# iamwangyabin/hardnetNas

Hardware: AMD Instinct MI355X
Metric: Mpatches/s (32×32→128-D) at 1/2/4/8 MI355X; HPatches FPR95 parity (higher is better)
Workload: dtype bf16x3; 1 GPU; Stock HardNet forward, 262144 synthetic 32x32 patches per GPU; model=hardnet, global_batch=262144, per_gpu_batch=262144, parallelism=dp1

## Files before the change

### hardnetnas_amd/csrc/hn_api.hip

```cpp
#include "hardnet_mi355x.h"
#include "hn_internal.h"

#include <algorithm>
#include <cmath>
#include <cstdlib>
#include <cstring>
#include <map>
#include <mutex>
#include <string>
#include <utility>
#include <vector>

static thread_local std::string g_err;

static int env_int(const char* name, int dflt) {
  const char* e = std::getenv(name);
  return e ? std::atoi(e) : dflt;
}

void hn_read_knobs(HnKnobs* k) {
  *k = HnKnobs{};
  k->c12_cfg = env_int("HN_C12_CFG", 15);
  k->head = std::getenv("HN_HEAD_V1") ? 1 : env_int("HN_HEAD", 4);
  k->head_pf = env_int("HN_HEAD_PF", 1) != 0;
  k->fdl_valu = std::getenv("HN_FDL_VALU") != nullptr;
  k->naive_pw = std::getenv("HN_NAIVE_PW") != nullptr;
  k->naive_dw = std::getenv("HN_NAIVE_DW") != nullptr;
  k->no_skipfuse = std::getenv("HN_NO_SKIPFUSE") != nullptr;
  k->no_irfskip = std::getenv("HN_NO_IRFSKIP") != nullptr;
  k->pairdist_valu = std::getenv("HN_PAIRDIST_VALU") != nullptr;
  k->pairdist_reg = env_int("HN_PAIRDIST_REG", 0) != 0;
  k->pairdist_spread = env_int("HN_PAIRDIST_SPREAD", 1) != 0;
  k->front_fold = env_int("HN_FRONT_FOLD", 0) != 0;
  k->u8_apart = env_int("HN_U8_APART", 0) != 0;
  k->front_xch3 = env_int("HN_FRONT_XCH3", 0) != 0;
  k->no_mpfront = env_int("HN_NO_MPFRONT", 0) != 0;
  k->pipeline = env_int("HN_PIPELINE", 0) != 0;

  k->train_splitk = std::max(32, env_int("HN_TRAIN_SPLITK", 1024)) / 32 * 32;
  k->train_f32 = env_int("HN_TRAIN_F32", 17) & 255;
#ifdef HN_EXPERIMENTS
  k->c12_abl = env_int("HN_C12_ABL", 0) & 4095;
  k->c12w_pd = env_int("HN_C12W_PD", 11);
  k->dbg = env_int("HN_DEBUG", 0);
  k->head_abl = env_int("HN_HEAD_ABL", 0);
  k->w4_abl = env_int("HN_W4_ABL", 0);
  k->pairdist_abl = env_int("HN_PAIRDIST_ABL", 0);
  k->irf3 = env_int("HN_IRF3", 0) != 0;
#endif
}

static thread_local const HnKnobs* tl_knobs = nullptr;

const HnKnobs& hn_knobs() {
  if (tl_knobs) return *tl_knobs;
  static std::once_flag once;
  static HnKnobs process;
  std::call_once(once, [] { hn_read_knobs(&process); });
  return process;
}

namespace {
struct KnobScope {
  const HnKnobs* prev;
  explicit KnobScope(const HnKnobs* k) : prev(tl_knobs) { tl_knobs = k; }
  ~KnobScope() { tl_knobs = prev; }
};
}

hipError_t hn_resident_blocks(const void* fn, int nthreads, int lds, int* resident) {
  static std::mutex mu;
  static std::map<std::pair<const void*, int>, int> cache;
  int dev = 0;
  hipError_t e = hipGetDevice(&dev);
  if (e != hipSuccess) return e;
  std::lock_guard<std::mutex> lock(mu);
  auto it = cache.find({fn, dev});
  if (it != cache.end()) {
    *resident = it->second;
    return hipSuccess;
  }
  if (lds > 0 && (e = hipFuncSetAttribute(fn, hipFuncAttributeMaxDynamicSharedMemorySize, lds)) != hipSuccess)
    return e;
  int per_cu = 0, cus = 0;
  if ((e = hipOccupancyMaxActiveBlocksPerMultiprocessor(&per_cu, fn, nthreads, lds)) != hipSuccess) return e;
  if ((e = hipDeviceGetAttribute(&cus, hipDeviceAttributeMultiprocessorCount, dev)) != hipSuccess) return e;
  const int r = std::max(1, per_cu) * std::max(1, cus);
  cache[{fn, dev}] = r;
  *resident = r;
  return hipSuccess;
}

static int fail(int code, const std::string& msg) {
  g_err = msg;
  return code;
}

#define HIPCHK(x)                                                                          \
  do {                                                                                     \
    hipError_t e_ = (x);                                                                   \
    if (e_ != hipSuccess)                                                                  \
      return fail(HN_ERR_HIP, std::string(#x) + ": " + hipGetErrorString(e_));             \
  } while (0)

const HnOpSpec kHnOps[17] = {
    {"skip", 1, 0, 0, 0, 0},        {"ir_k3_e1", 0, 1, 3, 1, 0},    {"ir_k3_e3", 0, 3, 3, 1, 0},
    {"ir_k3_s4", 0, 4, 3, 4, 0},    {"ir_k5_e1", 0, 1, 5, 1, 0},    {"ir_k5_e3", 0, 3, 5, 1, 0},
    {"ir_k5_s4", 0, 4, 5, 4, 0},    {"ir_k3_e1_se", 0, 1, 3, 1, 1}, {"ir_k3_e3_se", 0, 3, 3, 1, 1},
    {"ir_k3_s4_se", 0, 4, 3, 4, 1}, {"ir_k5_e1_se", 0, 1, 5, 1, 1}, {"ir_k5_e3_se", 0, 3, 5, 1, 1},
    {"ir_k5_s4_se", 0, 4, 5, 4, 1}, {"ir_k3_s2", 0, 1, 3, 2, 0},    {"ir_k5_s2", 0, 1, 5, 2, 0},
    {"ir_k3_s2_se", 0, 1, 3, 2, 1}, {"ir_k5_s2_se", 0, 1, 5, 2, 1},
};

namespace {

using OpSpec = HnOpSpec;
const OpSpec* const kOps = kHnOps;

struct NasLayer {
  int op = 0, cin = 0, cout = 0, stride = 1, hin = 0, hout = 0;
  int skip = 0, e = 1, k = 3, g = 1, se = 0, mid = 0, semid = 0;
  int skip_conv = 0;
  float *pw_w = nullptr, *pw_b = nullptr, *dw_w = nullptr, *dw_b = nullptr;
  float *pwl_w = nullptr, *pwl_b = nullptr;
  float *se_w1 = nullptr, *se_b1 = nullptr, *se_w2 = nullptr, *se_b2 = nullptr;
  uint16_t* front_a = nullptr;
  uint16_t* front_pwl16 = nullptr;
  float* front_b = nullptr;
  uint16_t *irf_pw_a = nullptr, *irf_pwl_a = nullptr;
  uint16_t* skip_a = nullptr;
  float* irf_pw_b = nullptr;
};

struct Cursor {
  const float* p;
  size_t n, i = 0;
  bool ok = true;
  const float* take(size_t k) {
    if (i + k > n) {
      ok = false;
      return nullptr;
    }
    const float* r = p + i;
    i += k;
    return r;
  }
};

uint16_t f2bf(float x) {
  uint32_t u;
  std::memcpy(&u, &x, 4);
  u += 0x7FFFu + ((u >> 16) & 1u);
  return (uint16_t)(u >> 16);
}
float bf2f(uint16_t b) {
  uint32_t u = (uint32_t)b << 16;
  float f;
  std::memcpy(&f, &u, 4);
  return f;
}

struct Folded {
  std::vector<float> w, b;
};
Folded fold(const float* w, size_t per_out, int cout, const float* gamma, const float* beta,
            const float* mean, const float* var, float eps) {
  Folded f;
  f.w.resize((size_t)cout * per_out);
  f.b.resize(cout);
  for (int n = 0; n < cout; ++n) {
    const double sc = (gamma ? (double)gamma[n] : 1.0) / std::sqrt((double)var[n] + (double)eps);
    for (size_t j = 0; j < per_out; ++j)
      f.w[(size_t)n * per_out + j] = (float)((double)w[(size_t)n * per_out + j] * sc);
    f.b[n] = (float)((beta ? (double)beta[n] : 0.0) - (double)mean[n] * sc);
  }
  return f;
}
// ... 1734 lines not shown
```

### hardnetnas_amd/csrc/hn_internal.h

```cpp
#pragma once
#include <hip/hip_runtime.h>

#include <algorithm>
#include <type_traits>

#include "hardnet_mi355x.h"

struct HnKnobs {
  int c12_cfg = 15;
  int head = 4;
  bool head_pf = true;
  bool fdl_valu = false;
  bool naive_pw = false;
  bool naive_dw = false;
  bool no_skipfuse = false;
  bool no_irfskip = false;
  bool pairdist_valu = false;
  bool pairdist_reg = false;
  bool pairdist_spread = true;
  bool front_fold = false;
  bool u8_apart = false;
  bool front_xch3 = false;
  bool no_mpfront = false;
  bool pipeline = false;
  bool irf3 = false;
  int train_splitk = 1024;
  int train_f32 = 17;
  int c12w_pd = 11;
  int c12_abl = 0;
  int head_abl = 0;
  int w4_abl = 0;
  int pairdist_abl = 0;
  int dbg = 0;
};
void hn_read_knobs(HnKnobs* k);
const HnKnobs& hn_knobs();

hipError_t hn_resident_blocks(const void* fn, int nthreads, int lds, int* resident);

struct HardnetDev {
  float* stem_w = nullptr;
  float* stem_b = nullptr;
  void* wpack[7] = {};
  float* bias[7] = {};
  void* c12_w1 = nullptr;
  void* c12_w2 = nullptr;
  void* c12_w1w = nullptr;
  void* wino[7] = {};
  void* wino1[7] = {};
  void* wino4[7] = {};
};
struct HnU8In {
  const uint8_t* in;
  int resize;
  int normalize;
  float mean, stdv;
};
hipError_t hn_launch_c12(const float* in, float* out, const HardnetDev& d, int P, float eps,
                         hipStream_t st, const HnU8In* u8 = nullptr);

hipError_t hn_launch_stem(const float* in, float* out, const float* w, const float* b, int P,
                          bool norm, float eps, hipStream_t st);
using HnConvLaunch = hipError_t (*)(const HardnetDev& d, const float* in, float* out, int P, float eps,
                                    hipStream_t st);
struct HnConvRow {
  int layer, variant;
  HnConvLaunch launch;
};
template <int N>
constexpr const HnConvRow* hn_find_row(const HnConvRow (&rows)[N], int layer, int variant) {
  for (const HnConvRow& r : rows)
    if (r.layer == layer && r.variant == variant) return &r;
  return nullptr;
}
template <int N>
constexpr bool hn_rows_unique(const HnConvRow (&rows)[N]) {
  for (int i = 0; i < N; ++i)
    if (hn_find_row(rows, rows[i].layer, rows[i].variant) != &rows[i]) return false;
  return true;
}
const HnConvRow* hn_hardnet_conv_row(int layer, int variant);
const HnConvRow* hn_wino1_conv_row(int layer, int variant);
const HnConvRow* hn_wino_conv_row(int layer, int variant);
bool hn_hardnet_variant_ok(int layer, int variant);

template <auto Kernel, int NTHR, int SMEM, class... Args>
hipError_t hn_launch_persistent(int tiles, hipStream_t st, Args... args) {
  int resident = 0;
  const hipError_t e = hn_resident_blocks(reinterpret_cast<const void*>(Kernel), NTHR, SMEM, &resident);
  if (e != hipSuccess) return e;
  const int grid = std::min(tiles, resident);
  if (grid <= 0) return hipSuccess;
  hipLaunchKernelGGL(Kernel, dim3(grid), dim3(NTHR), SMEM, st, args...);
  return hipGetLastError();
}

using HnC12Launch = hipError_t (*)(const float* in, float* out, const HardnetDev& d, int P, float eps,
                                   hipStream_t st, const HnU8In* u8);
constexpr int kAnyPd = -1;
struct HnC12Row {
  int cfg, abl, pd;
  HnC12Launch launch;
};
constexpr int kC12Wino = 14;
constexpr int kC12Split = 15;
template <int N>
constexpr const HnC12Row* hn_find_row(const HnC12Row (&rows)[N], int cfg, int abl, int pd) {
  for (const HnC12Row& r : rows)
    if (r.cfg == cfg && r.abl == abl && (r.pd == pd || r.pd == kAnyPd)) return &r;
  return nullptr;
}
template <int N>
constexpr bool hn_rows_unique(const HnC12Row (&rows)[N]) {
  for (int i = 0; i < N; ++i)
    if (hn_find_row(rows, rows[i].cfg, rows[i].abl, rows[i].pd) != &rows[i]) return false;
  return true;
}
const HnC12Row* hn_c12_row(int cfg, int abl, int pd);
const HnC12Row* hn_c12w_row(int cfg, int abl, int pd);
bool hn_c12_cfg_ok(int cfg, int abl, int pd);
template <auto Kernel, auto Base, int NTHR>
hipError_t hn_c12_launch(const void* w1, const float* in, float* out, const HardnetDev& d, int P, float eps,
                         hipStream_t st, const HnU8In* u8) {
  int resident = 0;
  const hipError_t e = hn_resident_blocks(reinterpret_cast<const void*>(Base), NTHR, 0, &resident);
  if (e != hipSuccess) return e;
  const int grid = (int)std::min<long>((long)P, resident);
  const void* src = u8 ? u8->in : static_cast<const void*>(in);
  hipLaunchKernelGGL(Kernel, dim3(grid), dim3(NTHR), 0, st, src, out, d.stem_w, d.stem_b, static_cast<const uint4*>(w1),
                     d.bias[1], static_cast<const uint4*>(d.c12_w2), d.bias[2], P, eps, u8 ? u8->mean : 0.f,
                     u8 ? u8->stdv : 1.f, u8 ? u8->normalize : 0);
  return hipGetLastError();
}
template <class F>
hipError_t hn_with_u8(const HnU8In* u8, F&& f) {
  if (!u8) return f(std::integral_constant<int, -1>{});
  switch (u8->resize) {
    case HN_RESIZE_NONE: return f(std::integral_constant<int, HN_RESIZE_NONE>{});
    case HN_RESIZE_CV2_LINEAR: return f(std::integral_constant<int, HN_RESIZE_CV2_LINEAR>{});
    case HN_RESIZE_PIL_BILINEAR: return f(std::integral_constant<int, HN_RESIZE_PIL_BILINEAR>{});
  }
  return hipErrorInvalidValue;
}
constexpr int kHeadSplitMaxP = 16384;
constexpr int head_split(int K) { return K / 128; }
hipError_t hn_launch_head(const float* a, float* out, const void* wp, const float* bias, int P,
                          int K, float l2eps, hipStream_t st, bool f16 = false, float* part = nullptr);
int hn_conv_lds_bytes(int layer);
hipError_t hn_launch_conv_raw(int layer, const void* wp, const float* zero_bias, const float* in, float* out,
                              int P, hipStream_t st);
int hn_wino1_lds_bytes(int layer);

hipError_t hn_launch_pw(const float* in, float* out, const float* wt, const float* bias,
                        const float* res, long npix, int cin, int cout, int groups, bool relu,
                        int shuffle_g, hipStream_t st);
hipError_t hn_launch_dw(const float* in, float* out, const float* wd, const float* bias, int P,
                        int hin, int c, int k, int s, hipStream_t st);
hipError_t hn_launch_maxpool(const float* in, float* out, int P, int hin, int c, hipStream_t st);
bool hn_skip_s2_supported(int hin, int cin, int cout);
hipError_t hn_launch_skip_s2(const float* in, float* out, const float* wt, const float* bias, int P, int hin,
                             int cin, int cout, hipStream_t st);
hipError_t hn_launch_se(float* y, const float* w1, const float* b1, const float* w2,
                        const float* b2, int P, int hw, int c, int mid, hipStream_t st);
hipError_t hn_launch_nas_head(const float* a, float* out, const float* wt, const float* bias,
// ... 156 lines not shown
```

### hardnetnas_amd/csrc/hn_wino1.hip

```cpp
#include "hn_common.h"
#include "hn_internal.h"

namespace {

template <int CIN, int COUT, int H, int NP, int WM, int WN, bool CST>
struct W1Cfg {
  static constexpr int TR = H;
  static constexpr int NTX = H / 2;
  static constexpr int BM = NP * TR * NTX;
  static constexpr int MT = BM / WM / 32, NT = COUT / WN / 32;
  static constexpr int NTOT = COUT / 32, NCC = CIN / 32;
  static constexpr int XROW = NTX * 64;
  static constexpr int RS = 4 * XROW;
  static constexpr int PS = TR * RS;
  static constexpr int ZROW = NP * PS;
  static constexpr int PLANE = ZROW + RS;
  static constexpr int BUF = 2 * PLANE;
  static constexpr int NWC = WM * WN, NWP = 4, NTHR = (NWC + NWP) * 64, PTHR = NWP * 64;
  static constexpr int UNITS = NP * TR * NTX * 4;
  static_assert(64 % (4 * NTX) == 0 && PTHR % (4 * NTX) == 0, "a row's units share one wave");
  static constexpr int UPT = (UNITS + PTHR - 1) / PTHR;
  static constexpr bool DEEP = UPT <= 2;
  static constexpr int SROW = 36;
  static constexpr int SCR_OFF = 2 * BUF;
  static constexpr int SCR = CST ? 32 * SROW * 4 : 0;
  static constexpr int BIAS_OFF = SCR_OFF + NWC * SCR;
  static constexpr int SMEM = BIAS_OFF + COUT * 4;
  static constexpr int NKS = 24;
  static constexpr unsigned CHUNK_BYTES = NKS * NTOT * 2 * 64 * 16;
  static_assert(SMEM <= 160 * 1024, "LDS");
  static_assert(MT >= 1 && NT >= 1 && MT * WM * 32 == BM && NT * WN * 32 == COUT, "tiling");
  static_assert((TR * NTX) % 32 == 0 && 32 % NTX == 0, "an M tile = 32 / NTX whole rows of one patch");
  static_assert(RS % 256 == 0, "image rows on 256-byte boundaries (the bank-conflict argument)");
};

template <int... I, class F>
HN_DEV void static_for_seq(std::integer_sequence<int, I...>, F&& f) {
  (f(std::integral_constant<int, I>{}), ...);
}
template <int N, class F>
HN_DEV void static_for(F&& f) {
  static_for_seq(std::make_integer_sequence<int, N>{}, f);
}

constexpr int w1_lo3(int g) { return g == 0 ? 0 : g == 1 ? 6 : g == 2 ? 11 : 16; }
constexpr int w1_fold_valu(bool first, int kx, int g) {
  if (kx == 11 && g >= 3) return 2 * (w1_lo3(g - 2) - w1_lo3(g - 3));
  if (kx == 12 && g < 3) return 2 * (w1_lo3(g + 1) - w1_lo3(g));
  if (kx == 18 || kx == 19 || (kx == 0 && !first)) return g < 5 ? 3 : 1;
  if (kx == 23 && g >= 3) return w1_lo3(g - 2) - w1_lo3(g - 3);
  return 0;
}

template <int CIN, int COUT, int H, int NP, int WM, int WN, bool CST, int WD = 3, int ABL = 0>
__global__ __launch_bounds__((WM * WN + 4) * 64) void k_conv_w1(const float* __restrict__ in, float* __restrict__ out,
                                                                const uint4* __restrict__ wp,
                                                                const float* __restrict__ bias, int P) {
  using C = W1Cfg<CIN, COUT, H, NP, WM, WN, CST>;
  constexpr int TR = C::TR;
  extern __shared__ __attribute__((aligned(16))) char smem[];
  const int tid = threadIdx.x, lane = tid & 63;
  const int wave = __builtin_amdgcn_readfirstlane(tid >> 6);
  const bool producer = wave >= C::NWC;
  const int r = lane & 31, h = lane >> 5;
  const int nwg = gridDim.x, rb = xcd_remap(blockIdx.x, nwg);
  const int ntiles = (P + NP - 1) / NP;
  const int my_tiles = rb < ntiles ? (ntiles - 1 - rb) / nwg + 1 : 0;
  const int NS = my_tiles * C::NCC;
  if (NS == 0) return;
  char* const buf0 = smem;
  char* const buf1 = smem + C::BUF;
  auto tile_of = [&](int s) { return (rb + (s / C::NCC) * nwg) * NP; };

  const int ptid = tid - C::NWC * 64;
  float4 pf[C::UPT][6], pf2[C::UPT][6];
  constexpr unsigned PATCH_BYTES = (unsigned)H * H * CIN * 4, OOB = 0x80000000u;
  auto produce_loads = [&](int s, float4 (&d)[C::UPT][6]) {
    const bool live = s < NS;
    const int p0 = live ? tile_of(s) : 0;
    const int cc = s % C::NCC;
    const int nval = !live ? 0 : P - p0 < NP ? P - p0 : NP;
    const __amdgpu_buffer_rsrc_t rs = make_rsrc(in + (size_t)p0 * H * H * CIN, (unsigned)nval * PATCH_BYTES);
#pragma unroll
    for (int k = 0; k < C::UPT; ++k) {
      const int u = ptid + k * C::PTHR;
      const int g = u & 3, t = (u >> 2) % C::NTX, rest = (u >> 2) / C::NTX;
      const int y = rest % TR, np = rest / TR;
      const bool rowok = C::UNITS % C::PTHR == 0 || u < C::UNITS;
#pragma unroll
      for (int j = 0; j < 3; ++j) {
        const int x = 2 * t - 1 + j;
        const bool ok = rowok && (j < 2 || t == C::NTX - 1) && (unsigned)x < (unsigned)H;
        const unsigned vo = ok ? (unsigned)(((np * H + y) * H + x) * CIN + cc * 32 + g * 8) * 4u : OOB;
        d[k][2 * j] = __builtin_bit_cast(float4, buf_load16(rs, vo, 0));
        d[k][2 * j + 1] = __builtin_bit_cast(float4, buf_load16(rs, vo, 16));
      }
    }
  };
  auto shfl4 = [&](const float4& v) {
    return make_float4(__shfl_down(v.x, 4, 64), __shfl_down(v.y, 4, 64), __shfl_down(v.z, 4, 64),
                       __shfl_down(v.w, 4, 64));
  };
  auto produce_write = [&](char* dst, const float4 (&d)[C::UPT][6]) {
#pragma unroll
    for (int k = 0; k < C::UPT; ++k) {
      const int u = ptid + k * C::PTHR;
      const int g = u & 3, t = (u >> 2) % C::NTX, rest = (u >> 2) / C::NTX;
      const int y = rest % TR, np = rest / TR;
      const bool last = t == C::NTX - 1;
      const float4 z = make_float4(0.f, 0.f, 0.f, 0.f);
      float4 dd[4][2];
#pragma unroll
      for (int i = 0; i < 2; ++i) {
        const float4 n0 = shfl4(d[k][i]), n1 = shfl4(d[k][2 + i]);
        dd[0][i] = d[k][i];
        dd[1][i] = d[k][2 + i];
        dd[2][i] = last ? d[k][4 + i] : n0;
        dd[3][i] = last ? z : n1;
      }
      if (C::UNITS % C::PTHR == 0 || u < C::UNITS) {
        const int off = np * C::PS + y * C::RS + t * 64 + 16 * (g ^ ((y + 1) & 3));
#pragma unroll
        for (int xi = 0; xi < 4; ++xi) {
          float4 v[2];
#pragma unroll
          for (int i = 0; i < 2; ++i) {
            const float4 d0 = dd[0][i], d1 = dd[1][i], d2 = dd[2][i], d3 = dd[3][i];
            if (xi == 0) v[i] = make_float4(d0.x - d2.x, d0.y - d2.y, d0.z - d2.z, d0.w - d2.w);
            if (xi == 1) v[i] = make_float4(d1.x + d2.x, d1.y + d2.y, d1.z + d2.z, d1.w + d2.w);
            if (xi == 2) v[i] = make_float4(d2.x - d1.x, d2.y - d1.y, d2.z - d1.z, d2.w - d1.w);
            if (xi == 3) v[i] = make_float4(d1.x - d3.x, d1.y - d3.y, d1.z - d3.z, d1.w - d3.w);
          }
          uint4 hi, lo;
          split8(v[0], v[1], hi, lo);
          *reinterpret_cast<uint4*>(dst + off + xi * C::XROW) = hi;
          *reinterpret_cast<uint4*>(dst + C::PLANE + off + xi * C::XROW) = lo;
        }
      }
    }
  };

  for (int i = tid; i < 4 * C::RS / 16; i += C::NTHR) {
    const int q = i / (C::RS / 16), o = (i % (C::RS / 16)) * 16;
    *reinterpret_cast<uint4*>(smem + (q >> 1) * C::BUF + (q & 1) * C::PLANE + C::ZROW + o) = make_uint4(0, 0, 0, 0);
  }
  if constexpr ((ABL & 64) != 0) {
    if (!producer) __builtin_amdgcn_s_setprio(1);
  }
  if constexpr ((ABL & 128) != 0) {
    if (producer) __builtin_amdgcn_s_setprio(1);
  }
  if (producer) {
    if constexpr ((ABL & 1) != 0) {
#pragma unroll 1
      for (int s = 0; s <= NS; ++s) __syncthreads();
      return;
    }
    produce_loads(0, pf);
    produce_write(buf0, pf);
    produce_loads(1, pf);
    __syncthreads();
    if constexpr (!C::DEEP) {
#pragma unroll 1
      for (int s = 0; s < NS; ++s) {
        produce_write((s & 1) ? buf0 : buf1, pf);
        produce_loads(s + 2, pf);
        __syncthreads();
      }
    } else {
#pragma unroll 1
      for (int s = 0; s < NS; s += 2) {
        produce_loads(s + 2, pf2);
        produce_write(buf1, pf);
        __syncthreads();
        if (s + 1 >= NS) break;
        produce_loads(s + 3, pf);
        produce_write(buf0, pf2);
        __syncthreads();
      }
    }
    return;
  }

  for (int i = tid; i < COUT; i += C::NWC * 64) reinterpret_cast<float*>(smem + C::BIAS_OFF)[i] = bias[i];
  __syncthreads();
  if constexpr ((ABL & 16) != 0) {
#pragma unroll 1
    for (int s = 0; s < NS; ++s) __syncthreads();
    return;
  }
  const int wm = wave / WN, wn = wave % WN;
  const float* const sbias = reinterpret_cast<const float*>(smem + C::BIAS_OFF);
  int ylr[C::MT], vo[C::MT][3][2];
#pragma unroll
  for (int mt = 0; mt < C::MT; ++mt) {
    const int m = (wm * C::MT + mt) * 32 + r;
    const int np = m / (TR * C::NTX), rem = m % (TR * C::NTX);
    ylr[mt] = rem / C::NTX;
#pragma unroll
    for (int ky = 0; ky < 3; ++ky) {
      const int wr = ylr[mt] + ky;
      const int rowb = (wr >= 1 && wr <= TR) ? np * C::PS + (wr - 1) * C::RS : C::ZROW;
#pragma unroll
      for (int ks = 0; ks < 2; ++ks) {
        vo[mt][ky][ks] = rowb + (rem % C::NTX) * 64 + 16 * ((2 * ks + h) ^ (wr & 3));
        asm volatile("" : "+v"(vo[mt][ky][ks]));
      }
    }
  }
  const __amdgpu_buffer_rsrc_t wr_ = make_rsrc(wp, C::NCC * C::CHUNK_BYTES);
  const unsigned wvoff = (wn * C::NT * 2 * 64 + lane) * 16;
  static_assert(C::MT * C::NT == 2, "the fold schedule below is written for two accumulator tiles per wave");
  f32x16 y0a[2], y1a[2], ma[2];

  auto load_b = [&](int cc, int kx, uint4 (&dst)[C::NT][2]) {
#pragma unroll
    for (int nt = 0; nt < C::NT; ++nt) {
      const unsigned k = cc * C::CHUNK_BYTES + (((ABL & 4) ? 0 : kx) * C::NTOT + nt) * 2 * 64 * 16;
      dst[nt][0] = buf_load16(wr_, wvoff, k);
      dst[nt][1] = buf_load16(wr_, wvoff, k + 64 * 16);
    }
  };
  static_assert(C::NKS % WD == 0, "the weight ring runs on across stages");
  uint4 bq[WD][C::NT][2];
#pragma unroll
  for (int k = 0; k + 1 < WD; ++k) load_b(0, k, bq[k]);

  auto sadd = [](float a, float b) {
    float v = a + b;
    asm("" : "+v"(v));
    return v;
  };
  auto ssub = [](float a, float b) {
    float v = a - b;
    asm("" : "+v"(v));
    return v;
  };
  auto fold = [&](auto first_, auto kx_, auto g_) {
    constexpr bool first = decltype(first_)::value;
    constexpr int kx = decltype(kx_)::value, g = decltype(g_)::value;
    if constexpr ((kx == 11 && g >= 3) || (kx == 12 && g < 3)) {
      constexpr int j = kx == 11 ? 0 : 1, g3 = kx == 11 ? g - 3 : g;
#pragma unroll
      for (int i = w1_lo3(g3); i < w1_lo3(g3 + 1); ++i) {
        y0a[j][i] = sadd(y0a[j][i], ma[j][i]);
        y1a[j][i] = sadd(first ? 0.f : y1a[j][i], ma[j][i]);
      }
    } else if constexpr (kx == 18 || kx == 19) {
#pragma unroll
      for (int i = 3 * g; i < 3 * g + 3 && i < 16; ++i) y0a[kx - 18][i] = sadd(y0a[kx - 18][i], ma[kx - 18][i]);
    } else if constexpr (kx == 23 && g >= 3) {
#pragma unroll
      for (int i = w1_lo3(g - 3); i < w1_lo3(g - 2); ++i) y1a[0][i] = ssub(y1a[0][i], ma[0][i]);
    } else if constexpr (kx == 0 && !first) {
#pragma unroll
      for (int i = 3 * g; i < 3 * g + 3 && i < 16; ++i) y1a[1][i] = ssub(y1a[1][i], ma[1][i]);
    }
  };

  auto stage = [&](auto first_, int s, int cc, int ccn) {
    constexpr bool FIRST = decltype(first_)::value;
    const char* cur = (s & 1) ? buf1 : buf0;
    uint4 aq[2][C::MT][2];
    auto load_a = [&](int kx, uint4 (&dst)[C::MT][2]) {
      const int xi = kx / 6, ky = (kx % 6) >> 1, ks = kx & 1;
#pragma unroll
      for (int mt = 0; mt < C::MT; ++mt) {
        const char* pa = cur + vo[mt][ky][ks];
        dst[mt][0] = *reinterpret_cast<const uint4*>(pa + xi * C::XROW);
        dst[mt][1] = *reinterpret_cast<const uint4*>(pa + (C::PLANE + xi * C::XROW));
      }
    };
    load_a(0, aq[0]);
    static_for<C::NKS>([&](auto kx_) {
      constexpr int kx = decltype(kx_)::value, xi = kx / 6;
      if constexpr ((ABL & 32) != 0) {
      } else if constexpr (kx + WD - 1 < C::NKS)
        load_b(cc, kx + WD - 1, bq[(kx + WD - 1) % WD]);
      else
        load_b(ccn, kx + WD - 1 - C::NKS, bq[(kx + WD - 1) % WD]);
      if constexpr (kx + 1 < C::NKS) load_a(kx + 1, aq[(kx + 1) & 1]);
      __builtin_amdgcn_sched_barrier(0);
      static_for<6>([&](auto g_) {
        constexpr int g = decltype(g_)::value, j = g / 3, p = g % 3, mt = j / C::NT, nt = j % C::NT;
        const bf16x8 x = as_bf16x8(aq[kx & 1][mt][p == 1 ? 1 : 0]), w = as_bf16x8(bq[kx % WD][nt][p == 0 ? 1 : 0]);
        f32x16& acc = xi == 0 ? y0a[j] : xi == 3 ? y1a[j] : ma[j];
        constexpr bool zero = p == 0 && (kx == 6 || kx == 12 || (kx == 0 && FIRST));
        if constexpr ((ABL & 2) != 0) {
          if (FIRST && kx == 0 && p == 0) y0a[j] = y1a[j] = ma[j] = f32x16{};
          if (p == 0)
            y0a[j][0] += __builtin_bit_cast(float, aq[kx & 1][mt][0].x ^ aq[kx & 1][mt][1].y ^
                                                       bq[kx % WD][nt][0].z ^ bq[kx % WD][nt][1].w);
        } else {
          acc = __builtin_amdgcn_mfma_f32_32x32x16_bf16(w, x, zero ? f32x16{} : acc, 0, 0, 0);
          constexpr int nv = w1_fold_valu(FIRST, kx, g);
          if constexpr (nv > 0) {
            fold(first_, kx_, g_);
            __builtin_amdgcn_sched_group_barrier(0x008, 1, 0);
            __builtin_amdgcn_sched_group_barrier(0x002, nv, 0);
          } else if constexpr (w1_fold_valu(FIRST, kx, 0) + w1_fold_valu(FIRST, kx, 5) > 0) {
            __builtin_amdgcn_sched_group_barrier(0x008, 1, 0);
          }
        }
      });
      __builtin_amdgcn_sched_barrier(0);
    });
  };
  auto fold_last = [&] {
#pragma unroll
    for (int i = 0; i < 16; ++i) y1a[1][i] = ssub(y1a[1][i], ma[1][i]);
  };
#pragma unroll 1
  for (int t = 0; t < my_tiles; ++t) {
    const int s0 = t * C::NCC, s = s0 + C::NCC - 1;
    stage(std::true_type{}, s0, 0, C::NCC > 1 ? 1 : 0);
#pragma unroll 1
    for (int cc = 1; cc < C::NCC; ++cc) {
      __syncthreads();
      stage(std::false_type{}, s0 + cc, cc, (cc + 1) % C::NCC);
    }
    if constexpr ((ABL & 2) == 0) fold_last();
    {
      const int p0 = tile_of(s);
      int le = lane;
      asm volatile("" : "+v"(le));
      const int r = le & 31, h = le >> 5;
#pragma unroll
      for (int nt = 0; nt < C::NT; ++nt) {
        float4 bv[4];
#pragma unroll
        for (int q = 0; q < 4; ++q)
          bv[q] = *reinterpret_cast<const float4*>(sbias + (wn * C::NT + nt) * 32 + 8 * q + 4 * h);
#pragma unroll
        for (int mt = 0; mt < C::MT; ++mt) {
          const int m0 = (wm * C::MT + mt) * 32;
          const int np = m0 / (TR * C::NTX), yb = (m0 % (TR * C::NTX)) / C::NTX;
          if ((NP == 1 || p0 + np < P) && ((ABL & 8) == 0 || y0a[mt * C::NT + nt][0] == 1234.5f)) {
            float* const ob = out + (((size_t)p0 + np) * H + yb) * H * COUT + (wn * C::NT + nt) * 32;
#pragma unroll
            for (int par = 0; par < 2; ++par) {
              const f32x16& yv = par ? y1a[mt * C::NT + nt] : y0a[mt * C::NT + nt];
              float4 v[4];
#pragma unroll
              for (int q = 0; q < 4; ++q)
                v[q] = make_float4(relu0(yv[4 * q + 0] + bv[q].x), relu0(yv[4 * q + 1] + bv[q].y),
                                   relu0(yv[4 * q + 2] + bv[q].z), relu0(yv[4 * q + 3] + bv[q].w));
              if constexpr (CST) {
                float* scr = reinterpret_cast<float*>(smem + C::SCR_OFF) + wave * (C::SCR / 4);
#pragma unroll
                for (int q = 0; q < 4; ++q) *reinterpret_cast<float4*>(scr + r * C::SROW + 8 * q + 4 * h) = v[q];
                __builtin_amdgcn_wave_barrier();
                asm volatile("" ::: "memory");
#pragma unroll
                for (int k = 0; k < 4; ++k) {
                  const int ml = 8 * k + (le >> 3), c4 = le & 7;
                  const int px = (ml / C::NTX) * H + 2 * (ml % C::NTX) + par;
                  *reinterpret_cast<float4*>(ob + (size_t)px * COUT + 4 * c4) =
                      *reinterpret_cast<const float4*>(scr + ml * C::SROW + 4 * c4);
                }
                __builtin_amdgcn_wave_barrier();
                asm volatile("" ::: "memory");
              } else {
                const int px = (r / C::NTX) * H + 2 * (r % C::NTX) + par;
#pragma unroll
                for (int q = 0; q < 4; ++q)
                  *reinterpret_cast<float4*>(ob + (size_t)px * COUT + 8 * q + 4 * h) = v[q];
              }
            }
          }
        }
      }
    }
    __syncthreads();
  }
}

template <int L, int CIN, int COUT, int H, int NP, int WM, int WN, bool CST, int WD, int ABL>
hipError_t launch_w1(const HardnetDev& d, const float* in, float* out, int P, float, hipStream_t st) {
  using C = W1Cfg<CIN, COUT, H, NP, WM, WN, CST>;
  if (!d.wino1[L]) return hipErrorInvalidValue;
  return hn_launch_persistent<&k_conv_w1<CIN, COUT, H, NP, WM, WN, CST, WD, ABL>, C::NTHR, C::SMEM>(
      (P + NP - 1) / NP, st, in, out, static_cast<const uint4*>(d.wino1[L]), d.bias[L], P);
}

#ifdef HN_EXPERIMENTS
template <int CIN, int COUT, int H, int NP, int WN>
struct W4Cfg {
  static constexpr int NTX = H / 4;
  static constexpr int POS = NP * H * NTX;
  static constexpr int MT = POS / 16;
  static constexpr int NCC = CIN / 32;
  static constexpr int NT = COUT / 16 / WN;
  static constexpr int RB = NTX * 64;
  static constexpr int HR = H + 2;
  static constexpr int XB = HR * RB;
  static constexpr int PLANE = NP * 6 * XB;
  static constexpr int BUF = 2 * PLANE;
  static constexpr int NWC = WN, NWP = 4, NTHR = (NWC + NWP) * 64, PTHR = NWP * 64;
  static constexpr int UNITS = NP * H * NTX * 4;
  static constexpr int UPT = UNITS / PTHR;
  static constexpr bool DEEP = UPT <= 2;
  static constexpr int SMEM = 2 * BUF;
  static constexpr int NKS = 18;
  static constexpr unsigned KSTEP_BYTES = (COUT / 16) * 2 * 64 * 16;
  static constexpr unsigned CHUNK_BYTES = NKS * KSTEP_BYTES;
  static_assert(RB == 256, "the bank-conflict argument assumes 256-byte image rows");
  static_assert(UNITS % PTHR == 0 && UPT >= 1, "whole units per producer thread");
  static_assert(POS % 16 == 0 && NT >= 1 && NT * WN * 16 == COUT, "tiling");
  static_assert(SMEM <= 160 * 1024, "LDS");
};

__host__ __device__ constexpr int w4_xi(int xo) { return xo == 0 ? 0 : xo == 1 ? 5 : xo - 1; }

template <int CIN, int COUT, int H, int NP, int WN, int WD, int ABL = 0>
__global__ __launch_bounds__((WN + 4) * 64) void k_conv_w4(const float* __restrict__ in, float* __restrict__ out,
                                                           const uint4* __restrict__ wp,
                                                           const float* __restrict__ bias, int P) {
  using C = W4Cfg<CIN, COUT, H, NP, WN>;
  constexpr int NTX = C::NTX;
  extern __shared__ __attribute__((aligned(16))) char smem[];
  const int tid = threadIdx.x, lane = tid & 63;
  const int wave = __builtin_amdgcn_readfirstlane(tid >> 6);
  const bool producer = wave >= C::NWC;
  const int nwg = gridDim.x, rb = xcd_remap(blockIdx.x, nwg);
  const int ntiles = (P + NP - 1) / NP;
  const int my_tiles = rb < ntiles ? (ntiles - 1 - rb) / nwg + 1 : 0;
  const int NS = my_tiles * C::NCC;
  if (NS == 0) return;
  char* const buf0 = smem;
  char* const buf1 = smem + C::BUF;
  auto tile_of = [&](int s) { return (rb + (s / C::NCC) * nwg) * NP; };

  constexpr int ZCH = C::RB / 16, NZ = 2 * 2 * NP * 6 * 2 * ZCH;
  for (int i = tid; i < NZ; i += C::NTHR) {
    const int q = i % ZCH, rest = i / ZCH;
    const int row = (rest & 1) ? C::HR - 1 : 0, blk = (rest >> 1) % (NP * 6), bp = (rest >> 1) / (NP * 6);
    *reinterpret_cast<uint4*>(smem + bp * C::PLANE + blk * C::XB + row * C::RB + q * 16) = make_uint4(0, 0, 0, 0);
  }

  if (producer) {
    if constexpr ((ABL & 1) != 0) {
#pragma unroll 1
      for (int s = 0; s <= NS; ++s) __syncthreads();
      return;
    }
    const int ptid = tid - C::NWC * 64;
    float4 pf[C::UPT][10], pf2[C::UPT][10];
    constexpr unsigned PATCH_BYTES = (unsigned)H * H * CIN * 4, OOB = 0x80000000u;
    auto produce_loads = [&](int s, float4 (&d)[C::UPT][10]) {
      const bool live = s < NS;
      const int p0 = live ? tile_of(s) : 0;
      const int cc = s % C::NCC;
      const int nval = !live ? 0 : P - p0 < NP ? P - p0 : NP;
      const __amdgpu_buffer_rsrc_t rs = make_rsrc(in + (size_t)p0 * H * H * CIN, (unsigned)nval * PATCH_BYTES);
#pragma unroll
      for (int k = 0; k < C::UPT; ++k) {
        const int u = ptid + k * C::PTHR;
        const int g = u & 3, t = (u >> 2) % NTX, rest = (u >> 2) / NTX;
        const int y = rest % H, np = rest / H;
#pragma unroll
        for (int j = 0; j < 5; ++j) {
          const int x = 4 * t - 1 + j;
          const bool ok = (j < 4 || t == NTX - 1) && (unsigned)x < (unsigned)H;
          const unsigned vo = ok ? (unsigned)(((np * H + y) * H + x) * CIN + cc * 32 + g * 8) * 4u : OOB;
          d[k][2 * j] = __builtin_bit_cast(float4, buf_load16(rs, vo, 0));
          d[k][2 * j + 1] = __builtin_bit_cast(float4, buf_load16(rs, vo, 16));
        }
      }
    };
    auto shfl4 = [&](const float4& v) {
      return make_float4(__shfl_down(v.x, 4, 64), __shfl_down(v.y, 4, 64), __shfl_down(v.z, 4, 64),
                         __shfl_down(v.w, 4, 64));
    };
    auto produce_write = [&](char* dst, const float4 (&d)[C::UPT][10]) {
#pragma unroll
      for (int k = 0; k < C::UPT; ++k) {
        const int u = ptid + k * C::PTHR;
        const int g = u & 3, t = (u >> 2) % NTX, rest = (u >> 2) / NTX;
        const int y = rest % H, np = rest / H;
        const bool last = t == NTX - 1;
        float4 dd[6][2];
#pragma unroll
        for (int i = 0; i < 2; ++i) {
          const float4 n0 = shfl4(d[k][i]), n1 = shfl4(d[k][2 + i]);
          dd[0][i] = d[k][i];
          dd[1][i] = d[k][2 + i];
          dd[2][i] = d[k][4 + i];
          dd[3][i] = d[k][6 + i];
          dd[4][i] = last ? d[k][8 + i] : n0;
          dd[5][i] = last ? make_float4(0.f, 0.f, 0.f, 0.f) : n1;
        }
        const int off = np * 6 * C::XB + (y + 1) * C::RB + t * 64 + 16 * (g ^ (2 * (y & 1)));
#pragma unroll
        for (int xi = 0; xi < 6; ++xi) {
          float4 v[2];
#pragma unroll
          for (int i = 0; i < 2; ++i) {
            auto tr = [&](float d0, float d1, float d2, float d3, float d4, float d5) {
              switch (xi) {
                case 0: return fmaf(0.25f, d0, fmaf(-1.25f, d2, d4));
                case 1: return fmaf(-0.25f, d1 + d2, d3 + d4);
                case 2: return fmaf(0.25f, d1 - d2, d4 - d3);
                case 3: return fmaf(-0.5f, d1 - d3, d4 - d2);
                case 4: return fmaf(0.5f, d1 - d3, d4 - d2);
                default: return fmaf(0.25f, d1, fmaf(-1.25f, d3, d5));
              }
            };
            v[i] = make_float4(tr(dd[0][i].x, dd[1][i].x, dd[2][i].x, dd[3][i].x, dd[4][i].x, dd[5][i].x),
                               tr(dd[0][i].y, dd[1][i].y, dd[2][i].y, dd[3][i].y, dd[4][i].y, dd[5][i].y),
                               tr(dd[0][i].z, dd[1][i].z, dd[2][i].z, dd[3][i].z, dd[4][i].z, dd[5][i].z),
                               tr(dd[0][i].w, dd[1][i].w, dd[2][i].w, dd[3][i].w, dd[4][i].w, dd[5][i].w));
          }
          uint4 hi, lo;
          split8(v[0], v[1], hi, lo);
          *reinterpret_cast<uint4*>(dst + off + xi * C::XB) = hi;
          *reinterpret_cast<uint4*>(dst + C::PLANE + off + xi * C::XB) = lo;
        }
      }
    };
    produce_loads(0, pf);
    produce_write(buf0, pf);
    produce_loads(1, pf);
    __syncthreads();
    if constexpr (!C::DEEP) {
#pragma unroll 1
      for (int s = 0; s < NS; ++s) {
        produce_write((s & 1) ? buf0 : buf1, pf);
        produce_loads(s + 2, pf);
        __syncthreads();
      }
    } else {
#pragma unroll 1
      for (int s = 0; s < NS; s += 2) {
// ... 231 lines not shown
```

Measured before the change: 5.532 Mpatches/s.

## Interleave Winograd conv epilogue stores into MFMA gaps of the last/next stage

Moves the bias+ReLU+LDS-transpose+global-store epilogue of the Winograd conv kernel into scheduled slots between MFMAs of the final channel stage (y0 half) and, for EPI=3, defers the y1 half into the next tile's first stage. Buffer stores with per-patch resource bounds replace the separate tail epilogue, hiding store latency behind matrix work. Adds register pressure and complex sched_group_barrier choreography, and is enabled by default via HN_W1_EPI except for one layer config.

```diff
diff --git a/hardnetnas_amd/csrc/hn_api.hip b/hardnetnas_amd/csrc/hn_api.hip
--- a/hardnetnas_amd/csrc/hn_api.hip
+++ b/hardnetnas_amd/csrc/hn_api.hip
@@ -23,6 +23,7 @@
   k->c12_cfg = env_int("HN_C12_CFG", 15);
   k->head = std::getenv("HN_HEAD_V1") ? 1 : env_int("HN_HEAD", 4);
   k->head_pf = env_int("HN_HEAD_PF", 1) != 0;
+  k->w1_epi = env_int("HN_W1_EPI", 1) != 0;
   k->fdl_valu = std::getenv("HN_FDL_VALU") != nullptr;
   k->naive_pw = std::getenv("HN_NAIVE_PW") != nullptr;
   k->naive_dw = std::getenv("HN_NAIVE_DW") != nullptr;
diff --git a/hardnetnas_amd/csrc/hn_internal.h b/hardnetnas_amd/csrc/hn_internal.h
--- a/hardnetnas_amd/csrc/hn_internal.h
+++ b/hardnetnas_amd/csrc/hn_internal.h
@@ -10,6 +10,7 @@
   int c12_cfg = 15;
   int head = 4;
   bool head_pf = true;
+  bool w1_epi = true;
   bool fdl_valu = false;
   bool naive_pw = false;
   bool naive_dw = false;
diff --git a/hardnetnas_amd/csrc/hn_wino1.hip b/hardnetnas_amd/csrc/hn_wino1.hip
--- a/hardnetnas_amd/csrc/hn_wino1.hip
+++ b/hardnetnas_amd/csrc/hn_wino1.hip
@@ -44,15 +44,25 @@
 }
 
 constexpr int w1_lo3(int g) { return g == 0 ? 0 : g == 1 ? 6 : g == 2 ? 11 : 16; }
-constexpr int w1_fold_valu(bool first, int kx, int g) {
+enum { W1_FIRST = 0, W1_PEND = 1, W1_MID = 2, W1_LAST = 3 };
+constexpr int w1_fold_valu(int mode, int kx, int g) {
   if (kx == 11 && g >= 3) return 2 * (w1_lo3(g - 2) - w1_lo3(g - 3));
   if (kx == 12 && g < 3) return 2 * (w1_lo3(g + 1) - w1_lo3(g));
-  if (kx == 18 || kx == 19 || (kx == 0 && !first)) return g < 5 ? 3 : 1;
+  if (kx == 18 || kx == 19 || (kx == 0 && mode != W1_FIRST)) return g < 5 ? 3 : 1;
   if (kx == 23 && g >= 3) return w1_lo3(g - 2) - w1_lo3(g - 3);
   return 0;
 }
-
-template <int CIN, int COUT, int H, int NP, int WM, int WN, bool CST, int WD = 3, int ABL = 0>
+constexpr int w1_epi_kx0(int mode) { return mode == W1_PEND ? 1 : mode == W1_LAST ? 20 : -1; }
+constexpr int w1_epi_slot(int mode, int kx, int g) {
+  const int kx0 = w1_epi_kx0(mode);
+  return kx0 >= 0 && kx >= kx0 && kx < kx0 + 4 ? (kx - kx0) * 6 + g : -1;
+}
+constexpr int w1_epi_valu(int e) { return e == 2 || e == 3 || e == 5 || e == 6 ? 8 : 0; }
+constexpr int w1_epi_dsw(int e) { return e == 3 || e == 4 || e == 6 || e == 7 ? 1 : 0; }
+constexpr int w1_epi_vst(int e) { return e == 9 || e == 11 ? 2 : 0; }
+constexpr int w1_epi_dsr(int e) { return e == 0 || e == 7 || e == 9 ? 2 : e == 2 || e == 3 ? 1 : 0; }
+
+template <int CIN, int COUT, int H, int NP, int WM, int WN, bool CST, int WD = 3, int ABL = 0, int EPI = 0>
 __global__ __launch_bounds__((WM * WN + 4) * 64) void k_conv_w1(const float* __restrict__ in, float* __restrict__ out,
                                                                 const uint4* __restrict__ wp,
                                                                 const float* __restrict__ bias, int P) {
@@ -236,8 +246,8 @@
     asm("" : "+v"(v));
     return v;
   };
-  auto fold = [&](auto first_, auto kx_, auto g_) {
-    constexpr bool first = decltype(first_)::value;
+  auto fold = [&](auto mode_, auto kx_, auto g_) {
+    constexpr bool first = decltype(mode_)::value <= W1_PEND, carry = decltype(mode_)::value != W1_FIRST;
     constexpr int kx = decltype(kx_)::value, g = decltype(g_)::value;
     if constexpr ((kx == 11 && g >= 3) || (kx == 12 && g < 3)) {
       constexpr int j = kx == 11 ? 0 : 1, g3 = kx == 11 ? g - 3 : g;
@@ -252,15 +262,84 @@
     } else if constexpr (kx == 23 && g >= 3) {
 #pragma unroll
       for (int i = w1_lo3(g - 3); i < w1_lo3(g - 2); ++i) y1a[0][i] = ssub(y1a[0][i], ma[0][i]);
-    } else if constexpr (kx == 0 && !first) {
+    } else if constexpr (kx == 0 && carry) {
 #pragma unroll
       for (int i = 3 * g; i < 3 * g + 3 && i < 16; ++i) y1a[1][i] = ssub(y1a[1][i], ma[1][i]);
     }
   };
 
-  auto stage = [&](auto first_, int s, int cc, int ccn) {
-    constexpr bool FIRST = decltype(first_)::value;
+  auto stage = [&](auto mode_, int s, int cc, int ccn, int ep0) __attribute__((always_inline)) {
+    constexpr int MODE = decltype(mode_)::value;
+    constexpr bool FIRST = MODE <= W1_PEND;
+    constexpr int EKX0 = EPI ? w1_epi_kx0(MODE) : -1, EPAR = MODE == W1_PEND ? 1 : 0;
+    static_assert(EPI || MODE == W1_FIRST || MODE == W1_MID, "the in-line epilogue has two stage forms");
+    static_assert(!EPI || (CST && 8 % C::NTX == 0 && C::NCC >= 2), "the gap epilogue's address terms");
     const char* cur = (s & 1) ? buf1 : buf0;
+    float4 T0, T1;
+    char *scw, *scr, *sbl;
+    unsigned svo;
+    __amdgpu_buffer_rsrc_t ers[2];
+    unsigned eso[2];
+    auto epi_setup = [&] {
+      int le = lane;
+      asm volatile("" : "+v"(le));
+      const int er = le & 31, eh = le >> 5, l3 = le >> 3, c4 = le & 7;
+      char* const sc = smem + C::SCR_OFF + wave * C::SCR;
+      scw = sc + (er * C::SROW + 4 * eh) * 4;
+      scr = sc + (l3 * C::SROW + 4 * c4) * 4;
+      sbl = smem + C::BIAS_OFF + (wn * C::NT * 32 + 4 * eh) * 4;
+      svo = (unsigned)((((l3 / C::NTX) * H + 2 * (l3 % C::NTX) + EPAR) * COUT + 4 * c4) * 4);
+#pragma unroll
+      for (int u = 0; u < 2; ++u) {
+        const int mt = u / C::NT, nt = u % C::NT;
+        const int m0 = (wm * C::MT + mt) * 32;
+        const int np = m0 / (TR * C::NTX), yb = (m0 % (TR * C::NTX)) / C::NTX;
+        constexpr unsigned PATCH_OUT = (unsigned)H * H * COUT * 4;
+        ers[u] = make_rsrc(out + ((size_t)ep0 + np) * H * H * COUT, NP == 1 || ep0 + np < P ? PATCH_OUT : 0u);
+        eso[u] = (unsigned)((yb * H * COUT + (wn * C::NT + nt) * 32) * 4);
+      }
+    };
+    auto epi = [&](auto u_, auto e_) {
+      constexpr int u = decltype(u_)::value, e = decltype(e_)::value, nt = u % C::NT;
+      f32x16& ya = MODE == W1_PEND ? y1a[u] : y0a[u];
+      auto ldb = [&](int q) { return *reinterpret_cast<const float4*>(sbl + nt * 128 + 32 * q); };
+      auto br = [&](int q, const float4& b) {
+        ya[4 * q + 0] = relu0(sadd(ya[4 * q + 0], b.x));
+        ya[4 * q + 1] = relu0(sadd(ya[4 * q + 1], b.y));
+        ya[4 * q + 2] = relu0(sadd(ya[4 * q + 2], b.z));
+        ya[4 * q + 3] = relu0(sadd(ya[4 * q + 3], b.w));
+      };
+      auto sw = [&](int q) {
+        *reinterpret_cast<float4*>(scw + 32 * q) = make_float4(ya[4 * q], ya[4 * q + 1], ya[4 * q + 2], ya[4 * q + 3]);
+      };
+      auto sr = [&](int k) { return *reinterpret_cast<const float4*>(scr + k * 8 * C::SROW * 4); };
+      auto st = [&](int k, const float4& v) {
+        buf_store16(ers[u], __builtin_bit_cast(uint4, v), svo, eso[u] + (unsigned)(k * (8 / C::NTX) * H * COUT * 4));
+      };
+      auto wbar = [] {
+        __builtin_amdgcn_wave_barrier();
+        asm volatile("" ::: "memory");
+      };
+      if constexpr (e == 0) {
+        T0 = ldb(0), T1 = ldb(1);
+      } else if constexpr (e == 2) {
+        br(0, T0), T0 = ldb(2);
+      } else if constexpr (e == 3) {
+        br(1, T1), T1 = ldb(3), sw(0);
+      } else if constexpr (e == 4) {
+        sw(1);
+      } else if constexpr (e == 5) {
+        br(2, T0);
+      } else if constexpr (e == 6) {
+        br(3, T1), sw(2);
+      } else if constexpr (e == 7) {
+        sw(3), wbar(), T0 = sr(0), T1 = sr(1);
+      } else if constexpr (e == 9) {
+        st(0, T0), st(1, T1), T0 = sr(2), T1 = sr(3);
+      } else if constexpr (e == 11) {
+        st(2, T0), st(3, T1), wbar();
+      }
+    };
     uint4 aq[2][C::MT][2];
     auto load_a = [&](int kx, uint4 (&dst)[C::MT][2]) {
       const int xi = kx / 6, ky = (kx % 6) >> 1, ks = kx & 1;
@@ -280,6 +359,7 @@
       else
         load_b(ccn, kx + WD - 1 - C::NKS, bq[(kx + WD - 1) % WD]);
       if constexpr (kx + 1 < C::NKS) load_a(kx + 1, aq[(kx + 1) & 1]);
+      if constexpr (kx == EKX0) epi_setup();
       __builtin_amdgcn_sched_barrier(0);
       static_for<6>([&](auto g_) {
         constexpr int g = decltype(g_)::value, j = g / 3, p = g % 3, mt = j / C::NT, nt = j % C::NT;
@@ -293,12 +373,19 @@
                                                        bq[kx % WD][nt][0].z ^ bq[kx % WD][nt][1].w);
         } else {
           acc = __builtin_amdgcn_mfma_f32_32x32x16_bf16(w, x, zero ? f32x16{} : acc, 0, 0, 0);
-          constexpr int nv = w1_fold_valu(FIRST, kx, g);
-          if constexpr (nv > 0) {
-            fold(first_, kx_, g_);
+          constexpr int nf = w1_fold_valu(MODE, kx, g), es = EPI ? w1_epi_slot(MODE, kx, g) : -1, e = es % 12;
+          constexpr int nv = nf + (es >= 0 ? w1_epi_valu(e) : 0);
+          if constexpr (nf > 0) fold(mode_, kx_, g_);
+          if constexpr (es >= 0) epi(std::integral_constant<int, es / 12>{}, std::integral_constant<int, e>{});
+          if constexpr (nv > 0 || es >= 0) {
             __builtin_amdgcn_sched_group_barrier(0x008, 1, 0);
-            __builtin_amdgcn_sched_group_barrier(0x002, nv, 0);
-          } else if constexpr (w1_fold_valu(FIRST, kx, 0) + w1_fold_valu(FIRST, kx, 5) > 0) {
+            if constexpr (nv > 0) __builtin_amdgcn_sched_group_barrier(0x002, nv, 0);
+            if constexpr (es >= 0) {
+              if constexpr (w1_epi_dsw(e) > 0) __builtin_amdgcn_sched_group_barrier(0x200, w1_epi_dsw(e), 0);
+              if constexpr (w1_epi_vst(e) > 0) __builtin_amdgcn_sched_group_barrier(0x040, w1_epi_vst(e), 0);
+              if constexpr (w1_epi_dsr(e) > 0) __builtin_amdgcn_sched_group_barrier(0x100, w1_epi_dsr(e), 0);
+            }
+          } else if constexpr (w1_fold_valu(MODE, kx, 0) + w1_fold_valu(MODE, kx, 5) > 0) {
             __builtin_amdgcn_sched_group_barrier(0x008, 1, 0);
           }
         }
@@ -310,18 +397,9 @@
 #pragma unroll
     for (int i = 0; i < 16; ++i) y1a[1][i] = ssub(y1a[1][i], ma[1][i]);
   };
-#pragma unroll 1
-  for (int t = 0; t < my_tiles; ++t) {
-    const int s0 = t * C::NCC, s = s0 + C::NCC - 1;
-    stage(std::true_type{}, s0, 0, C::NCC > 1 ? 1 : 0);
-#pragma unroll 1
-    for (int cc = 1; cc < C::NCC; ++cc) {
-      __syncthreads();
-      stage(std::false_type{}, s0 + cc, cc, (cc + 1) % C::NCC);
-    }
-    if constexpr ((ABL & 2) == 0) fold_last();
+  auto epilogue = [&](int p0, auto par0_, auto par1_) {
+    constexpr int PAR0 = decltype(par0_)::value, PAR1 = decltype(par1_)::value;
     {
-      const int p0 = tile_of(s);
       int le = lane;
       asm volatile("" : "+v"(le));
       const int r = le & 31, h = le >> 5;
@@ -338,7 +416,7 @@
           if ((NP == 1 || p0 + np < P) && ((ABL & 8) == 0 || y0a[mt * C::NT + nt][0] == 1234.5f)) {
             float* const ob = out + (((size_t)p0 + np) * H + yb) * H * COUT + (wn * C::NT + nt) * 32;
 #pragma unroll
-            for (int par = 0; par < 2; ++par) {
+            for (int par = PAR0; par < PAR1; ++par) {
               const f32x16& yv = par ? y1a[mt * C::NT + nt] : y0a[mt * C::NT + nt];
               float4 v[4];
 #pragma unroll
@@ -371,7 +449,58 @@
         }
       }
     }
-    __syncthreads();
+  };
+  using Mode = std::integral_constant<int, W1_FIRST>;
+  using ModePend = std::integral_constant<int, W1_PEND>;
+  using ModeMid = std::integral_constant<int, W1_MID>;
+  using ModeLast = std::integral_constant<int, W1_LAST>;
+  if constexpr (!EPI) {
+#pragma unroll 1
+    for (int t = 0; t < my_tiles; ++t) {
+      const int s0 = t * C::NCC, s = s0 + C::NCC - 1;
+      stage(Mode{}, s0, 0, C::NCC > 1 ? 1 : 0, 0);
+#pragma unroll 1
+      for (int cc = 1; cc < C::NCC; ++cc) {
+        __syncthreads();
+        stage(ModeMid{}, s0 + cc, cc, (cc + 1) % C::NCC, 0);
+      }
+      if constexpr ((ABL & 2) == 0) fold_last();
+      epilogue(tile_of(s), std::integral_constant<int, 0>{}, std::integral_constant<int, 2>{});
+      __syncthreads();
+    }
+  } else {
+    using I1 = std::integral_constant<int, 1>;
+    using I2 = std::integral_constant<int, 2>;
+    static_assert(EPI == 1 || EPI == 3, "bit 0: the y0 half in the last stage's gaps, bit 1: the y1 half deferred");
+    constexpr bool Y1D = (EPI & 2) != 0;
+    auto later_stages = [&](int s0) __attribute__((always_inline)) {
+#pragma unroll 1
+      for (int cc = 1; cc + 1 < C::NCC; ++cc) {
+        __syncthreads();
+        stage(ModeMid{}, s0 + cc, cc, cc + 1, 0);
+      }
+      __syncthreads();
+      stage(ModeLast{}, s0 + C::NCC - 1, C::NCC - 1, 0, tile_of(s0));
+      if constexpr (!Y1D) {
+        fold_last();
+        epilogue(tile_of(s0), I1{}, I2{});
+      }
+      __syncthreads();
+    };
+    stage(Mode{}, 0, 0, 1, 0);
+    later_stages(0);
+#pragma unroll 1
+    for (int t = 1; t < my_tiles; ++t) {
+      if constexpr (Y1D)
+        stage(ModePend{}, t * C::NCC, 0, 1, tile_of((t - 1) * C::NCC));
+      else
+        stage(Mode{}, t * C::NCC, 0, 1, 0);
+      later_stages(t * C::NCC);
+    }
+    if constexpr (Y1D) {
+      fold_last();
+      epilogue(tile_of(NS - 1), I1{}, I2{});
+    }
   }
 }
 
@@ -379,6 +508,11 @@
 hipError_t launch_w1(const HardnetDev& d, const float* in, float* out, int P, float, hipStream_t st) {
   using C = W1Cfg<CIN, COUT, H, NP, WM, WN, CST>;
   if (!d.wino1[L]) return hipErrorInvalidValue;
+  if constexpr (ABL == 0 && !(L == 5 && WD == 8)) {
+    if (hn_knobs().w1_epi)
+      return hn_launch_persistent<&k_conv_w1<CIN, COUT, H, NP, WM, WN, CST, WD, 0, L == 3 ? 1 : 3>, C::NTHR, C::SMEM>(
+          (P + NP - 1) / NP, st, in, out, static_cast<const uint4*>(d.wino1[L]), d.bias[L], P);
+  }
   return hn_launch_persistent<&k_conv_w1<CIN, COUT, H, NP, WM, WN, CST, WD, ABL>, C::NTHR, C::SMEM>(
       (P + NP - 1) / NP, st, in, out, static_cast<const uint4*>(d.wino1[L]), d.bias[L], P);
 }
```

Result: no change. 5.602 Mpatches/s (median of 6 runs) (+1.3%).
